# songrise/HyperNeRF-torch

Hardware: AMD Instinct MI355X
Metric: ray-samples/sec (fwd+bwd+Adam), whole job; per-GPU = value/n_gpus (higher is better)
Workload: dtype bf16

## Files before the change

### hypernerf-torch_amd/csrc/hn_mlp.hip

```cpp
#include "hn_common.h"
#include <algorithm>
#include <type_traits>

#ifdef HN_PROF
#define HN_STAMP(code)                                                                          \
  do {                                                                                          \
    if (prof_on && prof_n < 2040) {                                                             \
      unsigned long long t__;                                                                   \
      __builtin_amdgcn_sched_barrier(0);                                                        \
      asm volatile("s_memtime %0\n\ts_waitcnt lgkmcnt(0)" : "=s"(t__)::"memory");               \
      __builtin_amdgcn_sched_barrier(0);                                                        \
      if (lane == 0) { prof_buf[2 * prof_n] = (code); prof_buf[2 * prof_n + 1] = (long long)t__; } \
      ++prof_n;                                                                                 \
    }                                                                                           \
  } while (0)
#else
#define HN_STAMP(code) do {} while (0)
#endif

template <int WAVES>
struct WStream {
  const char* g;
  char* lds;
  int ctr;
// ... 463 lines not shown
#pragma unroll
  for (int t = 0; t <= NT; ++t) {
    const char* wl = nullptr;
    if (t < NT) wl = ws.take(N) + lane * 16;
    const int tp = t - 1;
    bf16x8 q[D];
    if (t < NT) {
      hn_init_acc(acc[t & 1], bias, t, h);
#pragma unroll
      for (int u = 0; u < D; ++u) q[u] = *reinterpret_cast<const bf16x8*>(wl + u * 1024);
    }
    __builtin_amdgcn_sched_barrier(0);
#pragma unroll
    for (int u = 0; u < N; ++u) {
      if (t < NT) {
        acc[t & 1] = hn_mfma_bf16(q[u % D], cur[u], acc[t & 1]);
        if (u + D < N) q[u % D] = *reinterpret_cast<const bf16x8*>(wl + (u + D) * 1024);
      }
      if (t > 0) {
#pragma unroll
        for (int e = 0; e < PER_SLOT; ++e) {
          const int k = u * PER_SLOT + e;
          if (k < SHARES)
            hn_epilogue_share<TRAIN, NT, S8>(k, tp, acc[tp & 1], nxt + tp * 2, bits, out_base, mask_base, lane);
        }
      }
      __builtin_amdgcn_sched_barrier(0);
    }
  }
#pragma unroll
  for (int i = 0; i < NT * 2; ++i) cur[i] = nxt[i];
}

template <bool BF16, int AUXG, bool EXTRA, bool TRAIN, bool S8 = false>
__global__ __launch_bounds__(ModeT<BF16>::WAVES * 64, BF16 ? 2 : 1) void hn_mlp_fwd_kernel(const HnMlpArgs a) {
  using M = ModeT<BF16>;
  constexpr int SX = S8 ? 1 : 0;
  static_assert(!(S8 && (EXTRA || !TRAIN || !BF16)), "the 8-bit stash exists for the render-level bf16 training builds only");
  if constexpr (S8) asm volatile("s_setreg_imm32_b32 hwreg(HW_REG_MODE, 23, 1), 1");
  using Frag = typename M::Frag;
  extern __shared__ __attribute__((aligned(16))) char smem[];
  const int lane = threadIdx.x & 63;
  const int wave = __builtin_amdgcn_readfirstlane(threadIdx.x >> 6);
  const int r = lane & 31, h = lane >> 5;
  constexpr int PTS = M::WAVES * 32;
  const int ntiles = (a.n_points + PTS - 1) / PTS;
  hn_timeline_begin(a.timeline);
#ifdef HN_PROF
  long long* prof_buf = reinterpret_cast<long long*>(a.prof);
  const bool prof_on = prof_buf != nullptr && blockIdx.x == 0 && wave == 0;
  int prof_n = 0;
#endif

  WStream<M::WAVES> ws;
  ws.g = reinterpret_cast<const char*>(a.wstream);
  ws.lds = smem;
  ws.nchunks = a.n_chunks;
  ws.wave = wave;
  ws.lane = lane;

  Frag cur[8 * M::STEPS32];
  Frag nxt[8 * M::STEPS32];

  float* bias_lds = reinterpret_cast<float*>(smem + 2 * HN_CHUNK_UNITS * 1024);
  HnFeat* feat_lds = reinterpret_cast<HnFeat*>(bias_lds + ((a.n_bias + 3) & ~3));
  HnDFeat* dfeat_lds = reinterpret_cast<HnDFeat*>(feat_lds + ((a.n_feat + 1) & ~1));
  const int n_trig = BF16 ? a.n_trig_comps : 0;
  const bool with_lo = a.trig_lo_planes != 0;
  const int n_planes = BF16 ? a.n_comps + n_trig + (with_lo ? n_trig : 1) : a.n_comps;
  float* srcv = reinterpret_cast<float*>(BF16 ? reinterpret_cast<char*>(dfeat_lds + a.n_feat)
                                              : reinterpret_cast<char*>(dfeat_lds)) + wave * (n_planes * 32);
  float* rev = BF16 ? srcv + a.n_comps * 32 : nullptr;
  for (int i = threadIdx.x; i < a.n_bias; i += blockDim.x) bias_lds[i] = a.bias[i];
  for (int i = threadIdx.x; i < a.n_feat; i += blockDim.x) {
    const HnFeat e = a.feat[i];
    feat_lds[i] = e;
    if constexpr (BF16) dfeat_lds[i] = hn_derive_feat_fwd(e, a.n_comps, n_trig, with_lo);
  }
  __syncthreads();

  for (int tile = blockIdx.x; tile < ntiles; tile += gridDim.x) {
    const int blk = tile * M::WAVES + wave;
    const int p0 = blk * 32 + r;
    const bool valid = p0 < a.n_points;
    const int p = valid ? p0 : a.n_points - 1;
    const int ray = p / a.samples_per_ray;
    const bool wave_valid = blk * 32 < a.n_points;
    hn_stage_sources(srcv, a, p, ray, lane, rev, n_trig, with_lo);
    ws.start();

    HnOpWords w_next = hn_load_op(a.ops, 0, a.n_ops);
    for (int op = 0; op < a.n_ops; ++op) {
      const HnOpWords w = w_next;
      w_next = hn_load_op(a.ops, op + 1, a.n_ops);
      const int code = w[0];
      if (code == HN_OP_LAYER) {
        HN_STAMP(100 + op);
        const int K32 = w[1] & 255, nG = (w[1] >> 8) & 255, NT = (w[1] >> 16) & 255;
        const int act = (w[1] >> 24) & 15, flags = (w[1] >> 28) & 15;
        const float* bias = bias_lds + w[2];
        const bool do_mask = TRAIN && w[4] >= 0 && wave_valid && act != HN_ACT_SOFTPLUS;
        const bool do_stash = TRAIN && w[5] >= 0 && wave_valid;
        char* out_base = do_stash ? hn_slot_base<BF16, SX>(a, w[5], NT, blk) : nullptr;
        char* aux_base = (TRAIN && wave_valid) ? hn_slot_base<BF16, SX>(a, w[6], 2 * nG, blk) : nullptr;
        uint32_t* mask_base = do_mask ? hn_mask_base(a, w[4], (NT + 1) >> 1, blk, lane) : nullptr;
        const bool has_out = w_next[0] == HN_OP_OUT;
        const HnOpWords out_w = w_next;
        Frag aux[AUXG * 2 * M::STEPS32];
#pragma unroll
        for (int g = 0; g < AUXG; ++g) {
          if (g < nG) {
            if (EXTRA && (flags & HN_LAYER_DIRECT))
              hn_make_group<true>(aux + g * 2 * M::STEPS32, feat_lds + w[3] + 64 * g, dfeat_lds + w[3] + 64 * g, srcv,
                                  lane, a, p, ray);
            else
              hn_make_group<false>(aux + g * 2 * M::STEPS32, feat_lds + w[3] + 64 * g, dfeat_lds + w[3] + 64 * g, srcv,
                                   lane, a, p, ray);
            if (aux_base != nullptr) {
              hn_stash<BF16, SX>(aux + g * 2 * M::STEPS32, aux_base, 2 * g, lane);
              hn_stash<BF16, SX>(aux + (g * 2 + 1) * M::STEPS32, aux_base, 2 * g + 1, lane);
            }
          }
        }
        unsigned bits = 0;
        HN_STAMP(1);
        if constexpr (BF16) {
          const bool plain = nG == 0 && act == HN_ACT_RELU && !(flags & HN_LAYER_NO_COMMIT) && !has_out &&
                             wave_valid && do_stash == do_mask;
          if (plain && K32 == 4 && NT == 4) {
            if (do_stash) hn_layer_pipelined<4, 4, true, SX>(cur, nxt, bias, ws, out_base, mask_base, lane);
            else hn_layer_pipelined<4, 4, false, SX>(cur, nxt, bias, ws, out_base, mask_base, lane);
            continue;
          }
        }
#pragma unroll
        for (int t = 0; t < 8; ++t) {
          if (t < NT) {
            f32x16 acc;
            hn_init_acc(acc, bias, t, h);
            hn_gemm_k<BF16>(acc, cur, K32, ws);
#pragma unroll
            for (int g = 0; g < AUXG; ++g)
              if (g < nG) hn_gemm_blocks<BF16, 2>(acc, aux + g * 2 * M::STEPS32, ws);
            HN_STAMP(2);
            if (act == HN_ACT_RELU) {
#pragma unroll
              for (int i = 0; i < 16; ++i) {
                bits = hn_push_mask<BF16>(bits, acc[i]);
                acc[i] = __int_as_float(max(__float_as_int(acc[i]), 0));
              }
            } else if (act != HN_ACT_NONE) {
              hn_act_tile<BF16>(acc, act, __int_as_float(w[7]), __int_as_float(w[4]), bits);
            }
            if (has_out && t == 0 && h == 0 && valid) {
              const HnDst d = a.dst[out_w[1]];
              const int n = out_w[3];
#pragma unroll
              for (int i = 0; i < 4; ++i) {
                if (i < n) {
                  float y = acc[i];
                  if (out_w[4] == 1) y = 1.0f / (1.0f + expf(-y));
                  if (out_w[5] >= 0) {
                    const HnSrc sr = a.src[out_w[5]];
                    y = __fadd_rn(sr.ptr[(size_t)(sr.per_ray ? ray : p) * sr.ld + out_w[6] + i], y);
                  }
                  d.ptr[(size_t)p * d.ld + out_w[2] + i] = y;
                }
              }
            }
            if (has_out && t == 0 && h == 0 && out_w[7] > 0) {
// ... 7 lines not shown
                    const HnSrc sr = a.src[out_w[5]];
                    y = __fadd_rn(sr.ptr[(size_t)(sr.per_ray ? ray : p) * sr.ld + out_w[6] + i], y);
                  }
                  const int ci = out_w[7] - 1 + i;
                  srcv[ci * 32 + r] = y;
                  if (BF16 && ci < n_trig) {
                    float hi, lo;
                    hn_rev_split(y, hi, lo);
                    rev[ci * 32 + r] = hi;
                    if (with_lo) rev[(n_trig + ci) * 32 + r] = lo;
                  }
                }
              }
            }
            hn_acc_to_frags(acc, nxt + t * M::STEPS32);
#ifdef HN_PROF
            if (prof_on) {
              float x__ = acc[15];
              asm volatile("v_mov_b32 %0, %0" : "+v"(x__)::"memory");
            }
#endif
            HN_STAMP(3);
            if ((t & 1) || t == NT - 1) {
              if (do_mask) mask_base[(t >> 1) * 64 + lane] = (t & 1) ? bits : bits << 16;
              bits = 0;
            }
            if (do_stash) {
              if constexpr (SX != 0) hn_stash8_acc<SX>(acc, out_base, t, lane);
              else hn_stash<BF16, SX>(nxt + t * M::STEPS32, out_base, t, lane);
            }
            HN_STAMP(4);
          }
        }
        if (!(flags & HN_LAYER_NO_COMMIT)) {
#pragma unroll
          for (int t = 0; t < 8; ++t)
            if (t < NT)
#pragma unroll
              for (int s = 0; s < M::STEPS32; ++s) cur[t * M::STEPS32 + s] = nxt[t * M::STEPS32 + s];
        }
      } else if (code == HN_OP_OUT) {
      } else if (EXTRA && code == HN_OP_OUT_WIDE) {
        const int n = w[3], NT = w[4];
        if (valid) {
          const HnDst d = a.dst[w[1]];
#pragma unroll
          for (int t = 0; t < 8; ++t)
            if (t < NT) {
              if constexpr (BF16) {
#pragma unroll
                for (int s = 0; s < 2; ++s)
#pragma unroll
                  for (int j = 0; j < 8; ++j) {
                    const int row = 32 * t + 16 * s + hn_pi16(h, j);
                    if (row < n) d.ptr[(size_t)p * d.ld + w[2] + row] = (float)cur[2 * t + s][j];
                  }
              } else {
#pragma unroll
                for (int q = 0; q < 16; ++q) {
                  const int row = 32 * t + hn_rho(q, h);
                  if (row < n) d.ptr[(size_t)p * d.ld + w[2] + row] = cur[16 * t + q];
                }
              }
            }
        }
      }
    }
  }
  hn_timeline_end(a.timeline);
}

HN_DEV bool hn_prefetch_masks(const HnMlpArgs& a, const HnOpWords& wn, int blk, int lane, bool wave_valid,
                              unsigned* out) {
  if (wn[0] != HN_BOP_LAYER || wn[4] < 0) return false;
  const int NT = (wn[1] >> 16) & 255;
  const uint32_t* mb = hn_mask_base(a, wn[4], (NT + 1) >> 1, blk, lane);
#pragma unroll
  for (int dd = 0; dd < 4; ++dd)
    out[dd] = (2 * dd < NT) ? (wave_valid ? mb[dd * 64 + lane] : 0xffffffffu) : 0u;
  return true;
}

template <bool BF16, bool WIDE, bool S8 = false>
__global__ __launch_bounds__(ModeT<BF16>::WAVES * 64, BF16 ? 2 : 1) void hn_mlp_bwd_kernel(const HnMlpArgs a) {
  using M = ModeT<BF16>;
  constexpr int SZ = S8 ? 2 : 0;
  static_assert(!(S8 && WIDE) && !(S8 && !BF16), "the 8-bit stash exists for the render-level bf16 builds only");
  if constexpr (S8) asm volatile("s_setreg_imm32_b32 hwreg(HW_REG_MODE, 23, 1), 1");
  const float dz_scale = S8 ? ldexpf(1.0f, a.dz_scale_log2) : 1.0f;
  const float dz_unscale = S8 ? ldexpf(1.0f, -a.dz_scale_log2) : 1.0f;
  using Frag = typename M::Frag;
  extern __shared__ __attribute__((aligned(16))) char smem[];
  const int lane = threadIdx.x & 63;
  const int wave = __builtin_amdgcn_readfirstlane(threadIdx.x >> 6);
  const int r = lane & 31, h = lane >> 5;
  constexpr int PTS = M::WAVES * 32;
  const int ntiles = (a.n_points + PTS - 1) / PTS;
  HnFeat* feat_lds = reinterpret_cast<HnFeat*>(smem + 2 * HN_CHUNK_UNITS * 1024);
  HnDFeat* dfeat_lds = reinterpret_cast<HnDFeat*>(feat_lds + ((a.n_feat + 1) & ~1));
  float* srcv = reinterpret_cast<float*>(BF16 ? reinterpret_cast<char*>(dfeat_lds + a.n_feat)
                                              : reinterpret_cast<char*>(dfeat_lds)) + wave * (a.n_comps * 32);
  hn_timeline_begin(a.timeline);
#ifdef HN_PROF
  long long* prof_buf = reinterpret_cast<long long*>(a.prof);
  const bool prof_on = prof_buf != nullptr && blockIdx.x == 0 && wave == 0;
  int prof_n = 0;
#endif
  for (int i = threadIdx.x; i < a.n_feat; i += blockDim.x) {
    const HnFeat e = a.feat[i];
    feat_lds[i] = e;
    if constexpr (BF16) dfeat_lds[i] = hn_derive_feat(e);
  }
  __syncthreads();

  WStream<M::WAVES> ws;
// ... 107 lines not shown
                float d = 1.0f;
                if (dact == HN_ACT_LEAKY_RELU) d = hn_keep_mask(nbits, t & 1, i) != 0 ? 1.0f : p0;
                else d = hn_dact_y<BF16>(dact, y[i], p0, p1);
                v[i] = g * d;
              }
            }
            hn_acc_to_frags(v, cur + t * M::STEPS32);
            if (dz_base != nullptr) hn_stash<BF16>(cur + t * M::STEPS32, dz_base, t, lane);
          }
        }
      } else if (code == HN_BOP_LAYER) {
        const int K32 = w[1] & 255, K32b = (w[1] >> 8) & 255, NT = (w[1] >> 16) & 255;
        const bool has_mask = w[4] >= 0;
        const bool do_stash = a.training && w[5] >= 0 && wave_valid;
        char* dz_base = do_stash ? hn_slot_base<BF16, SZ>(a, w[5], NT, blk) : nullptr;
        const int dact = w[2];
        const char* y_base = (!S8 && (dact == HN_ACT_ELU || dact == HN_ACT_SOFTPLUS) && wave_valid)
                                 ? hn_slot_base<BF16>(a, w[6], NT, blk) : nullptr;
        unsigned nbits = 0xffffffffu;
        unsigned mbits[4] = {0xffffffffu, 0xffffffffu, 0xffffffffu, 0xffffffffu};
        if (has_mask) {
          if (mnext_ready) {
#pragma unroll
            for (int dd = 0; dd < 4; ++dd) mbits[dd] = ~mnext[dd];
          } else {
            const uint32_t* mb = hn_mask_base(a, w[4], (NT + 1) >> 1, blk, lane);
#pragma unroll
            for (int dd = 0; dd < 4; ++dd)
              if (2 * dd < NT)
                mbits[dd] = wave_valid ? ~mb[dd * 64 + lane] : 0u;
          }
        }
        mnext_ready = false;
#pragma unroll
        for (int t = 0; t < 8; ++t) {
          if (t < NT) {
            f32x16 acc;
            hn_init_acc(acc, nullptr, t, h);
            hn_gemm_k<BF16>(acc, cur, K32, ws);
            if (K32b) hn_gemm_blocks<BF16, 1>(acc, cur2, ws);
            if (t == 0) mnext_ready = hn_prefetch_masks(a, w_next, blk, lane, wave_valid, mnext);
            HN_STAMP(2);
            if (!(t & 1)) nbits = mbits[t >> 1];
            if (dact == 0) {
#pragma unroll
              for (int i = 0; i < 16; ++i)
                acc[i] = __int_as_float(__float_as_int(acc[i]) & hn_keep_mask(nbits, t & 1, i));
            } else if (dact == HN_ACT_LEAKY_RELU) {
              const float p0 = __int_as_float(w[3]);
#pragma unroll
              for (int i = 0; i < 16; ++i)
                if (hn_keep_mask(nbits, t & 1, i) == 0) acc[i] *= p0;
            } else if (y_base != nullptr) {
              const f32x16 y = hn_unstash<BF16>(y_base, t, lane);
              const float p0 = __int_as_float(w[3]), p1 = __int_as_float(w[7]);
#pragma unroll
              for (int i = 0; i < 16; ++i) acc[i] *= hn_dact_y<BF16>(dact, y[i], p0, p1);
            }
            hn_acc_to_frags(acc, nxt + t * M::STEPS32);
            if (do_stash) {
              if constexpr (SZ != 0) hn_stash8_acc<SZ>(acc, dz_base, t, lane);
              else hn_stash<BF16, SZ>(nxt + t * M::STEPS32, dz_base, t, lane);
            }
            HN_STAMP(4);
          }
        }
// ... 569 lines not shown
    asm volatile("s_getreg_b32 %0, hwreg(HW_REG_HW_ID)" : "=s"(hw));
    asm volatile("s_getreg_b32 %0, hwreg(HW_REG_XCC_ID)" : "=s"(xcc));
    long long* o = jt_buf + (size_t)blockIdx.x * 8;
    o[0] = (long long)hw | ((long long)(xcc & 15u) << 32);
    o[1] = (long long)jt0; o[2] = (long long)jt1; o[3] = (long long)jt2; o[4] = (long long)wall_clock64();
    o[5] = (long long)nstage * (long long)stage_bytes; o[6] = jb.n_nt * 16 + jb.n_kt; o[7] = 1;
  }
#endif
  hn_timeline_end(tab.timeline);
}

static int hn_grid_for(int n_points, int pts_per_wg) {
  int tiles = (n_points + pts_per_wg - 1) / pts_per_wg;
  const int cap = 256 * 4;
  return tiles < cap ? tiles : cap;
}

extern "C" int hn_version(void) { return HN_VERSION; }

extern "C" int hn_abi_sizes(int32_t* out, int n) {
  const int32_t v[8] = {(int32_t)sizeof(HnMlpArgs),      (int32_t)sizeof(HnPackUnit), (int32_t)sizeof(HnPackBias),
                        (int32_t)sizeof(HnDwJob),        (int32_t)sizeof(HnCompositeArgs), (int32_t)sizeof(HnFeat),
                        (int32_t)sizeof(HnSlot),         (int32_t)sizeof(HnSrc)};
  static_assert(sizeof(HnDwBatch) == 40, "HnDwBatch layout");
  static_assert(sizeof(HnSrc) == 32, "HnSrc layout");
  for (int i = 0; i < n && i < 8; ++i) out[i] = v[i];
  return 8;
}

#define HN_STR2(x) #x
#define HN_STR(x) HN_STR2(x)
extern "C" __attribute__((used)) const char hn_build_config_text[] =
    "HN_BUILD_CONFIG:" HN_STR(HN_WGRAD_STAGES) "," HN_STR(HN_WGRAD_MAXSLOT) ",0," HN_STR(HN_CHUNK_UNITS) ",1,1,"
    HN_STR(HN_BF16_WAVES) "," HN_STR(HN_WGRAD_AUX) ";";
extern "C" int hn_build_config(int32_t* out, int n) {
  const int32_t v[HN_BUILD_CONFIG_N] = {HN_WGRAD_STAGES, HN_WGRAD_MAXSLOT, 0, HN_CHUNK_UNITS,
                                        1,               1,                HN_BF16_WAVES, HN_WGRAD_AUX};
  for (int i = 0; i < n && i < HN_BUILD_CONFIG_N; ++i) out[i] = v[i];
  return HN_BUILD_CONFIG_N;
}

static void hn_allow_big_lds() {
  static bool done[64] = {};
  int dev = 0;
  if (hipGetDevice(&dev) != hipSuccess || dev < 0 || dev >= 64) dev = 0;
  if (done[dev]) return;
  done[dev] = true;
  const int big = 160 * 1024;
#define HN_BIG(k) (void)hipFuncSetAttribute((const void*)(k), hipFuncAttributeMaxDynamicSharedMemorySize, big)
  HN_BIG((hn_mlp_fwd_kernel<true, 2, false, true>)); HN_BIG((hn_mlp_fwd_kernel<true, 2, false, false>));
  HN_BIG((hn_mlp_fwd_kernel<true, 2, true, true>)); HN_BIG((hn_mlp_fwd_kernel<true, 2, true, false>));
  HN_BIG((hn_mlp_fwd_kernel<true, 3, false, true>)); HN_BIG((hn_mlp_fwd_kernel<true, 3, false, false>));
  HN_BIG((hn_mlp_fwd_kernel<true, 3, true, true>)); HN_BIG((hn_mlp_fwd_kernel<true, 3, true, false>));
  HN_BIG((hn_mlp_fwd_kernel<false, 3, true, true>)); HN_BIG((hn_mlp_fwd_kernel<false, 3, true, false>));
  HN_BIG((hn_mlp_fwd_kernel<true, 2, false, true, true>)); HN_BIG((hn_mlp_fwd_kernel<true, 3, false, true, true>));
  HN_BIG((hn_mlp_bwd_kernel<true, false, true>)); HN_BIG((hn_wgrad_kernel<true, true>));
#undef HN_BIG
  (void)hipFuncSetAttribute((const void*)hn_mlp_bwd_kernel<true, false>, hipFuncAttributeMaxDynamicSharedMemorySize, big);
  (void)hipFuncSetAttribute((const void*)hn_mlp_bwd_kernel<true, true>, hipFuncAttributeMaxDynamicSharedMemorySize, big);
  (void)hipFuncSetAttribute((const void*)hn_mlp_bwd_kernel<false, true>, hipFuncAttributeMaxDynamicSharedMemorySize, big);
  (void)hipFuncSetAttribute((const void*)hn_wgrad_kernel<true>, hipFuncAttributeMaxDynamicSharedMemorySize, big);
  (void)hipFuncSetAttribute((const void*)hn_wgrad_kernel<false>, hipFuncAttributeMaxDynamicSharedMemorySize, big);
}

extern "C" int hn_pack_units(int mode, const HnPackUnit* units, int n_units, const float* const* ptrs, void* wstream,
                             const HnPackBias* bias, int n_bias, float* bias_out, hnStream_t stream) {
  if (n_units < 0 || n_bias < 0) return -1;
  const int total = n_units + n_bias;
  if (total == 0) return 0;
  const int grid = (total + 3) / 4;
// ... 530 lines not shown
```

### hypernerf-torch_amd/machine.py

```python
from __future__ import annotations

import os
import weakref

import ctypes as C
import itertools
import math
from dataclasses import dataclass, field
from typing import Dict, List, Optional, Sequence, Tuple

import numpy as np
import torch

from . import _lib as L

CHUNK = L.HN_CHUNK_UNITS


def pow2ceil(n: int) -> int:
    p = 1
    while p < n:
        p *= 2
    return p


def bf16_like(mode: int) -> bool:
    return mode in (L.HN_MODE_BF16, L.HN_MODE_BF16_S8)


def mode_consts(mode: int):
    if mode == L.HN_MODE_BF16_S8:
        return 2, 1024
    return (2, 2048) if mode == L.HN_MODE_BF16 else (4, 4096)


DZ_SCALE_LOG2 = int(os.environ.get("HN_DZ_SCALE_LOG2", 16))


ACT_CODES = {"none": L.HN_ACT_NONE, "relu": L.HN_ACT_RELU, "leaky_relu": L.HN_ACT_LEAKY_RELU, "elu": L.HN_ACT_ELU,
             "softplus": L.HN_ACT_SOFTPLUS}
MASK_ACTS = ("relu", "leaky_relu")
Y_ACTS = ("elu", "softplus")


def f32_bits(x: float) -> int:
    return int(np.array([x], dtype=np.float32).view(np.int32)[0])


@dataclass
class Feature:
    src: int
    comp: int
    kind: int
    freq: float = 1.0
    need_grad: bool = False


def posenc_features(src: int, comps: Sequence[int], n_freqs: int, need_grad: bool = False) -> List[Feature]:
    out = [Feature(src, c, L.HN_FEAT_ID, 1.0, need_grad) for c in comps]
    for k in range(n_freqs):
        f = float(2.0 ** k)
        out += [Feature(src, c, L.HN_FEAT_SIN, f, need_grad) for c in comps]
        out += [Feature(src, c, L.HN_FEAT_COS, f, need_grad) for c in comps]
    return out


def posenc_jax_features(src: int, comps: Sequence[int], min_deg: int, max_deg: int, use_identity: bool,
                        need_grad: bool = False) -> List[Feature]:
    steps = max_deg - min_deg
# ... 520 lines not shown
            if s.kind == "stash":
                offs.append((stash_b, s.nt))
                stash_b += nblk * s.nt * tile_bytes
            else:
                offs.append((mask_b, s.nt))
                mask_b += nblk * s.nt * 64 * 4
        return offs, stash_b, mask_b

    def resolved_ops(self, mode: int, n_points: int) -> Tuple[np.ndarray, np.ndarray]:
        offs, _, _ = self.layout(mode, n_points)

        def res(slot: int) -> int:
            if slot < 0:
                return -1
            off = offs[slot][0]
            unit = 1024 if self.slots[slot].kind == "stash" else 256
            assert off % unit == 0 and off // unit < 2 ** 31
            return off // unit
        fwd = self.fwd_ops.copy()
        for w in fwd:
            if w[0] == L.HN_OP_LAYER:
                if (int(w[1]) >> 24) & 15 != L.HN_ACT_SOFTPLUS:
                    w[4] = res(int(w[4]))
                w[5], w[6] = res(int(w[5])), res(int(w[6]))
        bwd = self.bwd_ops.copy()
        for w in bwd:
            if w[0] == L.HN_BOP_LOAD:
                w[7] = res(int(w[7]))
            elif w[0] == L.HN_BOP_LOAD_WIDE:
                if (int(w[3]) >> 16) & 15 != L.HN_ACT_SOFTPLUS:
                    w[5] = res(int(w[5]))
                w[7] = res(int(w[7]))
            elif w[0] == L.HN_BOP_LAYER:
                w[4], w[5] = res(int(w[4])), res(int(w[5]))
                if int(w[2]) in (L.HN_ACT_ELU, L.HN_ACT_SOFTPLUS):
                    w[6] = res(int(w[6]))
        return fwd, bwd

    def grad_offsets(self) -> Tuple[List[int], int]:
        offs, tot = [], 0
        for p in self.params:
            offs.append(tot)
            tot += (p.numel() + 3) // 4 * 4
        return offs, tot

    @staticmethod
    def _wave_grid(n_nt: int, n_kt: int, one_row: bool = False) -> Tuple[int, int]:
        if one_row:
            if n_nt <= 4:
                return 1, min(8, max(1, n_kt)) if n_kt <= 8 else 8
            return 2, 4
        best = None
        for gn in range(1, 9):
            for gk in range(1, 8 // gn + 1):
                if gn > n_nt or gk > n_kt:
                    continue
                tn, tk = -(-n_nt // gn), -(-n_kt // gk)
                if tn > 4 or tk > 2:
                    continue
                key = (-(gn * gk), tn * tk, gn * gk * (tn + tk))
                if best is None or key < best[0]:
                    best = (key, gn, gk)
        if best is None:
            raise NotImplementedError(f"no wave grid for a {n_nt} x {n_kt} tile rectangle")
        return best[1], best[2]

    def _wgrad_rects(self, mode: int, n_points: int) -> list:
        offs, _, _ = self.layout(mode, n_points)
        tmax = 8 if bf16_like(mode) else 4
        rects = []
        for ly in self.layers:
# ... 541 lines not shown
        a.masks = masks.data_ptr() if masks is not None else 0
        a.dsrc = dsrc.data_ptr() if dsrc is not None else 0
        for i, s in enumerate(srcs):
            if s is None:
                continue
            t, per_ray = s[0], s[1]
            L.require_gpu(t)
            if t.dtype != torch.float32 or t.stride(-1) != 1:
                raise L.HnError("sources must be fp32 with unit inner stride")
            a.src[i].ptr, a.src[i].ld, a.src[i].per_ray = t.data_ptr(), t.stride(-2) if t.dim() > 1 else 1, int(per_ray)
            if len(s) > 2 and s[2] is not None:
                idx = s[2]
                L.require_gpu(idx)
                if idx.dtype != torch.int64 or not idx.is_contiguous():
                    raise L.HnError("gather indices must be contiguous int64")
                a.src[i].gather_idx, a.src[i].gather_rows = idx.data_ptr(), t.shape[0]
        if embed is not None:
            g_tab, idx, src_i = embed[:3]
            if len(embed) > 3 and embed[3] is not None:
                a.embed_partial = embed[3].data_ptr()
            mask, col = self.prog.embed_fold(src_i)
            a.embed_reg_mask, a.embed_grad, a.embed_idx = mask, g_tab.data_ptr(), idx.data_ptr()
            a.embed_rows, a.embed_dim = g_tab.shape[0], g_tab.shape[1]
            for k in range(L.HN_DSRC_COMPS):
                a.embed_col[k] = col[k]
        for i, t in enumerate(dsts):
            if t is None:
                continue
            L.require_gpu(t)
            a.dst[i].ptr, a.dst[i].ld = t.data_ptr(), t.stride(-2) if t.dim() > 1 else 1
        return a

    def _ops(self, device, mode, n_points):
        key = ("ops", str(device), mode, n_points)
        hit = self._jobs.get(key)
        if hit is None:
            fwd, bwd = self.prog.resolved_ops(mode, n_points)
            hit = (L.to_device_bytes(fwd, device), L.to_device_bytes(bwd, device))
            self._jobs[key] = hit
        return hit

    @staticmethod
    def _job_bytes(mode: int) -> int:
        return WGRAD_JOB_BYTES // 2 if mode == L.HN_MODE_BF16_S8 else WGRAD_JOB_BYTES

    def effective_mode(self, mode: int) -> int:
        if mode == L.HN_MODE_BF16_S8:
            wide = any(ly.out is not None and ly.out.wide for ly in self.prog.layers)
            direct = any(f.kind != L.HN_FEAT_ZERO and (f.src, f.comp) not in self.prog.comp_map
                         for f in self.prog.feat_table)
            if wide or direct:
                return L.HN_MODE_BF16
        return mode

    def forward(self, mode, n_points, samples_per_ray, srcs, dsts, training: bool):
        mode = self.effective_mode(mode)
        if mode == L.HN_MODE_BF16_S8 and training and self.prog.y_acts:
            raise NotImplementedError(
                f"{self.prog.name}: precision 'bf16s8' keeps the training stash in 8 bits, too coarse to take the "
                "derivative of an ELU / Softplus layer from its output; use 'bf16' or 'fp32' (LeakyReLU works: it needs "
                "only the mask)")
        device = dsts[0].device if dsts and dsts[0] is not None else srcs[0][0].device
        d = self.pack(device, mode, force=training)
        stash = masks = None
        if training:
            _, sb, mb = self.prog.layout(mode, n_points)
            stash = torch.empty(max(sb, 16), dtype=torch.uint8, device=device)
# ... 67 lines not shown
```

### include/hn_kernels.h

```cpp
#ifndef HN_KERNELS_H
#define HN_KERNELS_H

#include <stdint.h>

#ifdef __cplusplus
extern "C" {
#endif

typedef void* hnStream_t;

#define HN_VERSION 340

#define HN_MODE_F32 0
#define HN_MODE_BF16 1
#define HN_MODE_BF16_S8 2

#define HN_MAX_SRC 8
#define HN_MAX_DST 4
#define HN_MAX_SLOTS 128
#define HN_OP_WORDS 8
#ifndef HN_CHUNK_UNITS
#define HN_CHUNK_UNITS 32
#endif
#define HN_DSRC_COMPS 32

#define HN_OP_LAYER 1
#define HN_ACT_NONE 0
#define HN_ACT_RELU 1
#define HN_ACT_LEAKY_RELU 2
#define HN_ACT_ELU 3
#define HN_ACT_SOFTPLUS 4
#define HN_LAYER_NO_COMMIT 1
#define HN_LAYER_DIRECT 2
#define HN_OP_OUT 4
#define HN_OP_OUT_WIDE 5

#define HN_BOP_LOAD 1
#define HN_BOP_LOAD_WIDE 2
#define HN_BOP_LAYER 3
#define HN_BOP_AUX 4

typedef struct {
  int32_t packed;
  float freq;
} HnFeat;
#define HN_MAX_COMPS 32
#define HN_FEAT_ID_DIRECT 5
#define HN_FEAT_ZERO 0
#define HN_FEAT_ID 1
#define HN_FEAT_SIN 2
#define HN_FEAT_COS 3
#define HN_FEAT_SINP 4

typedef struct {
  const float* ptr;
  int32_t ld;
  int32_t per_ray;
  const int64_t* gather_idx;
  int32_t gather_rows;
  int32_t pad;
} HnSrc;

typedef struct {
  float* ptr;
  int32_t ld;
  int32_t pad;
} HnDst;

typedef struct {
  uint64_t off;
  int32_t nt;
  int32_t pad;
// ... 43 lines not shown
  int32_t r_end;
  int32_t c_end;
  int32_t k0;
  int32_t transposed;
} HnPackUnit;

typedef struct {
  int32_t w_id;
  int32_t n;
  int32_t off;
  int32_t len;
} HnPackBias;

typedef struct {
  uint64_t z_off, x_off;
  int32_t z_nt, x_nt;
  int32_t z_t0, x_t0;
  int32_t n_nt, n_kt;
  int32_t blk0, blk1;
  int32_t w_off;
  int32_t ld;
  int32_t r0, c0;
  int32_t r_end, c_end;
  int32_t b_off;
  int32_t pad;
  uint64_t x2_off;
  int32_t x2_nt, x2_t0;
  int32_t n_kt1;
  int32_t p_tile;
} HnDwJob;

int hn_version(void);
int hn_abi_sizes(int32_t* out, int n);
#define HN_BUILD_CONFIG_N 8
int hn_build_config(int32_t* out, int n);

int hn_pack_units(int mode, const HnPackUnit* units_dev, int n_units, const float* const* ptrs_dev,
                  void* wstream_dev, const HnPackBias* bias_dev, int n_bias, float* bias_out_dev,
                  hnStream_t stream);

#define HN_MAX_PACK_JOBS 8
typedef struct {
  const HnPackUnit* units;
  const float* const* ptrs;
  void* wstream;
  const HnPackBias* bias;
  float* bias_out;
  int32_t n_units, n_bias;
} HnPackJob;
int hn_pack_units_multi(int mode, const HnPackJob* jobs_host, int n_jobs, hnStream_t stream);

int hn_mlp_forward(const HnMlpArgs* args, hnStream_t stream);
int hn_mlp_backward(const HnMlpArgs* args, hnStream_t stream);
int hn_mlp_workspace_bytes(const int32_t* ops_host, int n_ops, int backward, int mode, int64_t n_points,
                           int64_t* stash_bytes, int64_t* mask_bytes);

int hn_mlp_wgrad(int mode, const HnDwJob* jobs_dev, int n_jobs, const void* stash_dev,
                 float* grad_base_dev, hnStream_t stream);

#define HN_MAX_WGRAD_BATCH 8
typedef struct {
  const HnDwJob* jobs;
  const void* stash;
  float* grads;
  int32_t n_jobs;
  int32_t pad;
  float* partials;
// ... 206 lines not shown
```

### hypernerf-torch_amd/_lib.py

```python
from __future__ import annotations

import ctypes as C
import os
import subprocess

import numpy as np
import torch

_HERE = os.path.dirname(os.path.abspath(__file__))
CSRC = os.path.join(_HERE, "csrc")
PRODUCT_LIB_PATH = os.path.join(CSRC, "libhn_hip.so")
LIB_PATH = os.environ.get("HN_LIB_PATH") or PRODUCT_LIB_PATH
SOURCES = ["hn_mlp.hip", "hn_render.hip", "hn_calib.hip", "hn_optim.hip", "hn_metrics.hip"]
CSRC_HEADERS = ["hn_common.h", "hn_pack.h"]
HEADER = os.path.join(os.path.dirname(_HERE), "include", "hn_kernels.h")
BUILD_MACROS = ("HN_REDUCE_SPLIT", "HN_BF16_WAVES", "HN_PROF", "HN_CHUNK_UNITS", "HN_WGRAD_AUX", "HN_WGRAD_STAGES", "HN_WGRAD_MAXSLOT")

HN_MODE_F32, HN_MODE_BF16, HN_MODE_BF16_S8 = 0, 1, 2
BUILD_CONFIG_KEYS = ("WGRAD_STAGES", "WGRAD_MAXSLOT", "WGRAD_BIAS_MFMA", "CHUNK_UNITS", "WGRAD_BLOCK", "WSTREAM_ASYM",
                     "BF16_WAVES", "WGRAD_AUX")


def _read_build_config(path: str):
    import re
    try:
        with open(path, "rb") as f:
            blob = f.read()
    except OSError:
        return None
    m = re.search(rb"HN_BUILD_CONFIG:([0-9, ]+);", blob)
    if m is None:
        return None
    vals = [int(x) for x in m.group(1).decode().replace(" ", "").split(",")]
    return {k: v for k, v in zip(BUILD_CONFIG_KEYS, vals)}


BUILD_CONFIG = _read_build_config(LIB_PATH)
_cfg = BUILD_CONFIG or {}
WGRAD_STAGES = _cfg.get("WGRAD_STAGES", int(os.environ.get("HN_WGRAD_STAGES") or 2))
WGRAD_MAXSLOT = _cfg.get("WGRAD_MAXSLOT", int(os.environ.get("HN_WGRAD_MAXSLOT") or 8))
WGRAD_MAX_STAGE_KB = min(8 * WGRAD_MAXSLOT, 160 // WGRAD_STAGES)
HN_MAX_SRC, HN_MAX_DST, HN_MAX_SLOTS = 8, 4, 128
HN_OP_WORDS, HN_CHUNK_UNITS, HN_DSRC_COMPS = 8, _cfg.get("CHUNK_UNITS", int(os.environ.get("HN_CHUNK_UNITS", 32))), 32
HN_AUXG_MAX = 3
HN_MAX_COMPS = 32

HN_OP_LAYER, HN_OP_OUT, HN_OP_OUT_WIDE = 1, 4, 5
HN_ACT_NONE, HN_ACT_RELU, HN_ACT_LEAKY_RELU, HN_ACT_ELU, HN_ACT_SOFTPLUS = 0, 1, 2, 3, 4
HN_LAYER_NO_COMMIT, HN_LAYER_DIRECT = 1, 2
HN_BOP_LOAD, HN_BOP_LOAD_WIDE, HN_BOP_LAYER, HN_BOP_AUX = 1, 2, 3, 4
HN_FEAT_ZERO, HN_FEAT_ID, HN_FEAT_SIN, HN_FEAT_COS, HN_FEAT_SINP, HN_FEAT_ID_DIRECT = 0, 1, 2, 3, 4, 5


# ... 281 lines not shown
```

Measured before the change: 83.62 million.

## Software-pipeline backward ReLU layer epilogue with next tile's MFMA chain

Adds a specialized backward path for bf16 layers with K32=4, NT=4, ReLU-style masking (dact=0) and stashing. Each tile's mask, bf16 conversion and stash epilogue is interleaved with the next tile's MFMA chain, using double-buffered accumulators and a two-deep weight prefetch, with sched_barriers to fix the ordering. The intent is to hide epilogue ALU and LDS/global latency behind matrix-core work. The trade-off is higher register pressure, and an env var plus an op flag bit let the path be disabled.

```diff
diff --git a/hypernerf-torch_amd/csrc/hn_mlp.hip b/hypernerf-torch_amd/csrc/hn_mlp.hip
--- a/hypernerf-torch_amd/csrc/hn_mlp.hip
+++ b/hypernerf-torch_amd/csrc/hn_mlp.hip
@@ -745,6 +745,65 @@
   return true;
 }
 
+template <bool TRAIN, int SZ>
+HN_DEV void hn_bwd_epilogue_share(int k, int tp, f32x16& a, bf16x8* frag, unsigned nbits, char* dz_base, int lane) {
+  if (k < 8) {
+#pragma unroll
+    for (int e = 0; e < 2; ++e) {
+      const int i = 2 * k + e;
+      a[i] = __int_as_float(__float_as_int(a[i]) & hn_keep_mask(nbits, tp & 1, i));
+      frag[i >> 3][i & 7] = (__bf16)a[i];
+    }
+  } else if (TRAIN && k == 8) {
+    if constexpr (SZ != 0) hn_stash8_acc<SZ>(a, dz_base, tp, lane);
+    else hn_stash<true, 0>(frag, dz_base, tp, lane);
+  }
+}
+
+template <int K32, int NT, bool TRAIN, int SZ>
+HN_DEV bool hn_bwd_layer_pipelined(bf16x8* cur, bf16x8* nxt, const unsigned* mbits, WStream<ModeT<true>::WAVES>& ws,
+                                   char* dz_base, const HnMlpArgs& a, const HnOpWords& w_next, int blk, int lane,
+                                   unsigned* mnext) {
+  constexpr int N = 2 * K32;
+  constexpr int D = 2;
+  static_assert(8 % N == 0, "the eight element-pair shares are dealt evenly over the slots");
+  constexpr int PER_SLOT = 8 / N;
+  f32x16 acc[2];
+  bool mnext_ready = false;
+#pragma unroll
+  for (int t = 0; t <= NT; ++t) {
+    const char* wl = nullptr;
+    if (t < NT) wl = ws.take(N) + lane * 16;
+    if (t == 0) mnext_ready = hn_prefetch_masks(a, w_next, blk, lane, true, mnext);
+    const int tp = t - 1;
+    bf16x8 q[D];
+    if (t < NT) {
+      hn_init_acc(acc[t & 1], nullptr, t, 0);
+#pragma unroll
+      for (int u = 0; u < D; ++u) q[u] = *reinterpret_cast<const bf16x8*>(wl + u * 1024);
+    }
+    __builtin_amdgcn_sched_barrier(0);
+#pragma unroll
+    for (int u = 0; u < N; ++u) {
+      if (t < NT) {
+        acc[t & 1] = hn_mfma_bf16(q[u % D], cur[u], acc[t & 1]);
+        if (u + D < N) q[u % D] = *reinterpret_cast<const bf16x8*>(wl + (u + D) * 1024);
+      }
+      if (t > 0) {
+#pragma unroll
+        for (int e = 0; e < PER_SLOT; ++e)
+          hn_bwd_epilogue_share<TRAIN, SZ>(u * PER_SLOT + e, tp, acc[tp & 1], nxt + tp * 2, mbits[tp >> 1], dz_base, lane);
+        if (u == N - 1)
+          hn_bwd_epilogue_share<TRAIN, SZ>(8, tp, acc[tp & 1], nxt + tp * 2, mbits[tp >> 1], dz_base, lane);
+      }
+      __builtin_amdgcn_sched_barrier(0);
+    }
+  }
+#pragma unroll
+  for (int i = 0; i < NT * 2; ++i) cur[i] = nxt[i];
+  return mnext_ready;
+}
+
 template <bool BF16, bool WIDE, bool S8 = false>
 __global__ __launch_bounds__(ModeT<BF16>::WAVES * 64, BF16 ? 2 : 1) void hn_mlp_bwd_kernel(const HnMlpArgs a) {
   using M = ModeT<BF16>;
@@ -918,6 +977,12 @@
           }
         }
         mnext_ready = false;
+        if constexpr (BF16) {
+          if (!(w[1] & HN_BOP_GENERIC_ONLY) && K32b == 0 && dact == 0 && wave_valid && do_stash && K32 == 4 && NT == 4) {
+            mnext_ready = hn_bwd_layer_pipelined<4, 4, true, SZ>(cur, nxt, mbits, ws, dz_base, a, w_next, blk, lane, mnext);
+            continue;
+          }
+        }
 #pragma unroll
         for (int t = 0; t < 8; ++t) {
           if (t < NT) {
diff --git a/hypernerf-torch_amd/machine.py b/hypernerf-torch_amd/machine.py
--- a/hypernerf-torch_amd/machine.py
+++ b/hypernerf-torch_amd/machine.py
@@ -35,6 +35,9 @@
 
 
 DZ_SCALE_LOG2 = int(os.environ.get("HN_DZ_SCALE_LOG2", 16))
+
+BWD_PIPELINE = os.environ.get("HN_BWD_PIPE", "1") != "0"
+BOP_GENERIC_ONLY = -(1 << 31)
 
 
 ACT_CODES = {"none": L.HN_ACT_NONE, "relu": L.HN_ACT_RELU, "leaky_relu": L.HN_ACT_LEAKY_RELU, "elu": L.HN_ACT_ELU,
@@ -621,6 +624,8 @@
                     w[5] = res(int(w[5]))
                 w[7] = res(int(w[7]))
             elif w[0] == L.HN_BOP_LAYER:
+                if not BWD_PIPELINE:
+                    w[1] = int(w[1]) | BOP_GENERIC_ONLY
                 w[4], w[5] = res(int(w[4])), res(int(w[5]))
                 if int(w[2]) in (L.HN_ACT_ELU, L.HN_ACT_SOFTPLUS):
                     w[6] = res(int(w[6]))
@@ -1233,7 +1238,7 @@
         return a
 
     def _ops(self, device, mode, n_points):
-        key = ("ops", str(device), mode, n_points)
+        key = ("ops", str(device), mode, n_points, BWD_PIPELINE)
         hit = self._jobs.get(key)
         if hit is None:
             fwd, bwd = self.prog.resolved_ops(mode, n_points)
diff --git a/include/hn_kernels.h b/include/hn_kernels.h
--- a/include/hn_kernels.h
+++ b/include/hn_kernels.h
@@ -38,6 +38,7 @@
 #define HN_BOP_LOAD 1
 #define HN_BOP_LOAD_WIDE 2
 #define HN_BOP_LAYER 3
+#define HN_BOP_GENERIC_ONLY ((int)0x80000000)
 #define HN_BOP_AUX 4
 
 typedef struct {
```

Result: no change. 83.43 million (-0.2%).

## Add specialized fused trunk-layer paths for 256x256 ReLU layers in fwd and bwd

Applied to the files above, without the earlier changes.

Adds dedicated device routines for the common 8x8-tile ReLU trunk layers in the MLP forward and backward kernels. In the forward pass, two consecutive trunk layers run back to back with ping-pong buffers, so the copy between them is skipped. In the backward pass, a specialized masked-gradient loop replaces the generic one. The path is gated by a build macro that defaults on, and the macro is recorded in the build config. Costs include more code size and register pressure, which could hurt occupancy.

```diff
diff --git a/hypernerf-torch_amd/_lib.py b/hypernerf-torch_amd/_lib.py
--- a/hypernerf-torch_amd/_lib.py
+++ b/hypernerf-torch_amd/_lib.py
@@ -14,11 +14,11 @@
 SOURCES = ["hn_mlp.hip", "hn_render.hip", "hn_calib.hip", "hn_optim.hip", "hn_metrics.hip"]
 CSRC_HEADERS = ["hn_common.h", "hn_pack.h"]
 HEADER = os.path.join(os.path.dirname(_HERE), "include", "hn_kernels.h")
-BUILD_MACROS = ("HN_REDUCE_SPLIT", "HN_BF16_WAVES", "HN_PROF", "HN_CHUNK_UNITS", "HN_WGRAD_AUX", "HN_WGRAD_STAGES", "HN_WGRAD_MAXSLOT")
+BUILD_MACROS = ("HN_REDUCE_SPLIT", "HN_BF16_WAVES", "HN_PROF", "HN_CHUNK_UNITS", "HN_WGRAD_AUX", "HN_WGRAD_STAGES", "HN_WGRAD_MAXSLOT", "HN_TRUNK_BODY")
 
 HN_MODE_F32, HN_MODE_BF16, HN_MODE_BF16_S8 = 0, 1, 2
 BUILD_CONFIG_KEYS = ("WGRAD_STAGES", "WGRAD_MAXSLOT", "WGRAD_BIAS_MFMA", "CHUNK_UNITS", "WGRAD_BLOCK", "WSTREAM_ASYM",
-                     "BF16_WAVES", "WGRAD_AUX")
+                     "BF16_WAVES", "WGRAD_AUX", "TRUNK_BODY")
 
 
 def _read_build_config(path: str):
diff --git a/hypernerf-torch_amd/csrc/hn_mlp.hip b/hypernerf-torch_amd/csrc/hn_mlp.hip
--- a/hypernerf-torch_amd/csrc/hn_mlp.hip
+++ b/hypernerf-torch_amd/csrc/hn_mlp.hip
@@ -519,6 +519,65 @@
   for (int i = 0; i < NT * 2; ++i) cur[i] = nxt[i];
 }
 
+#ifndef HN_TRUNK_BODY
+#define HN_TRUNK_BODY 1
+#endif
+typedef __attribute__((ext_vector_type(8))) short hn_s16x8;
+template <bool TRAIN>
+HN_DEV bool hn_trunk_fwd_op(const HnOpWords& w, const HnOpWords& wn) {
+  constexpr int shape = 8 | 0 << 8 | 8 << 16 | HN_ACT_RELU << 24;
+  return w[0] == HN_OP_LAYER && (w[1] & 0x1fffffff) == shape && wn[0] != HN_OP_OUT &&
+         (!TRAIN || (w[4] >= 0) == (w[5] >= 0));
+}
+HN_DEV bool hn_trunk_bwd_op(const HnOpWords& w) {
+  return w[0] == HN_BOP_LAYER && w[1] == (8 | 8 << 16) && w[2] == 0 && w[4] >= 0;
+}
+template <bool TRAIN, int S8>
+HN_DEV void hn_trunk_fwd(const bf16x8* in, bf16x8* out, const float* bias, WStream<ModeT<true>::WAVES>& ws, bool store,
+                         char* out_base, uint32_t* mask_base, int lane) {
+  asm volatile("" : "+v"(lane));
+  const int h = lane >> 5;
+  unsigned bits = 0;
+#pragma unroll
+  for (int t = 0; t < 8; ++t) {
+    f32x16 acc;
+    hn_init_acc(acc, bias, t, h);
+    hn_gemm_blocks<true, 8>(acc, in, ws);
+    if constexpr (TRAIN) {
+#pragma unroll
+      for (int i = 0; i < 16; ++i) bits = hn_push_mask<true>(bits, acc[i]);
+    }
+#pragma unroll
+    for (int i = 0; i < 16; ++i) acc[i] = __int_as_float(max(__float_as_int(acc[i]), 0));
+    hn_acc_to_frags(acc, out + 2 * t);
+    if (TRAIN && store) {
+      if constexpr (S8 != 0) hn_stash8_acc<S8>(acc, out_base, t, lane);
+      else hn_stash<true, 0>(out + 2 * t, out_base, t, lane);
+    }
+    if (TRAIN && store && (t & 1)) mask_base[(t >> 1) * 64 + lane] = bits;
+  }
+}
+template <int S8, class F>
+HN_DEV void hn_trunk_bwd(const bf16x8* in, bf16x8* out, WStream<ModeT<true>::WAVES>& ws, const unsigned* mbits,
+                         bool store, char* dz_base, int lane, F&& after_first) {
+  asm volatile("" : "+v"(lane));
+#pragma unroll
+  for (int t = 0; t < 8; ++t) {
+    f32x16 acc;
+    hn_init_acc(acc, nullptr, t, 0);
+    hn_gemm_blocks<true, 8>(acc, in, ws);
+    if (t == 0) after_first();
+    const unsigned nbits = mbits[t >> 1];
+#pragma unroll
+    for (int i = 0; i < 16; ++i) acc[i] = __int_as_float(__float_as_int(acc[i]) & hn_keep_mask(nbits, t & 1, i));
+    hn_acc_to_frags(acc, out + 2 * t);
+    if (store) {
+      if constexpr (S8 != 0) hn_stash8_acc<S8>(acc, dz_base, t, lane);
+      else hn_stash<true, 0>(out + 2 * t, dz_base, t, lane);
+    }
+  }
+}
+
 template <bool BF16, int AUXG, bool EXTRA, bool TRAIN, bool S8 = false>
 __global__ __launch_bounds__(ModeT<BF16>::WAVES * 64, BF16 ? 2 : 1) void hn_mlp_fwd_kernel(const HnMlpArgs a) {
   using M = ModeT<BF16>;
@@ -566,12 +625,19 @@
   }
   __syncthreads();
 
+  constexpr bool TRUNK = HN_TRUNK_BODY && BF16 && TRAIN && !EXTRA && !S8 && AUXG == 2;
   for (int tile = blockIdx.x; tile < ntiles; tile += gridDim.x) {
+    int spr = a.samples_per_ray;
+    if constexpr (TRUNK) {
+      asm volatile("" : "+s"(spr));
+      asm volatile("v_mbcnt_lo_u32_b32 %0, -1, 0\n\tv_mbcnt_hi_u32_b32 %0, -1, %0" : "=&v"(ws.lane));
+    }
+    const int lane = ws.lane, r = lane & 31, h = lane >> 5;
     const int blk = tile * M::WAVES + wave;
     const int p0 = blk * 32 + r;
     const bool valid = p0 < a.n_points;
     const int p = valid ? p0 : a.n_points - 1;
-    const int ray = p / a.samples_per_ray;
+    const int ray = p / spr;
     const bool wave_valid = blk * 32 < a.n_points;
     hn_stage_sources(srcv, a, p, ray, lane, rev, n_trig, with_lo);
     ws.start();
@@ -620,9 +686,27 @@
             continue;
           }
         }
+        bool trunk = false, swapped = false;
+        if constexpr (TRUNK) {
+          trunk = wave_valid && hn_trunk_fwd_op<TRAIN>(w, w_next);
+          if (trunk) {
+            const HnOpWords w2 = hn_load_op(a.ops, op + 2, a.n_ops);
+            hn_trunk_fwd<TRAIN, SX>(cur, nxt, bias, ws, do_stash, out_base, mask_base, lane);
+            if (hn_trunk_fwd_op<TRAIN>(w_next, w2)) {
+              const bool st2 = TRAIN && w_next[5] >= 0;
+              char* ob2 = st2 ? hn_slot_base<true, SX>(a, w_next[5], 8, blk) : nullptr;
+              uint32_t* mb2 = st2 ? hn_mask_base(a, w_next[4], 4, blk, lane) : nullptr;
+              HN_STAMP(100 + op + 1);
+              hn_trunk_fwd<TRAIN, SX>(nxt, cur, bias_lds + w_next[2], ws, st2, ob2, mb2, lane);
+              ++op;
+              w_next = w2;
+              swapped = true;
+            }
+          }
+        }
 #pragma unroll
         for (int t = 0; t < 8; ++t) {
-          if (t < NT) {
+          if (t < NT && !trunk) {
             f32x16 acc;
             hn_init_acc(acc, bias, t, h);
             hn_gemm_k<BF16>(acc, cur, K32, ws);
@@ -696,7 +780,7 @@
             HN_STAMP(4);
           }
         }
-        if (!(flags & HN_LAYER_NO_COMMIT)) {
+        if (!(flags & HN_LAYER_NO_COMMIT) && !swapped) {
 #pragma unroll
           for (int t = 0; t < 8; ++t)
             if (t < NT)
@@ -918,6 +1002,17 @@
           }
         }
         mnext_ready = false;
+#if HN_TRUNK_BODY
+        if constexpr (BF16) {
+          if (hn_trunk_bwd_op(w)) {
+            hn_trunk_bwd<SZ>(cur, nxt, ws, mbits, do_stash, dz_base, lane,
+                             [&] { mnext_ready = hn_prefetch_masks(a, w_next, blk, lane, wave_valid, mnext); });
+#pragma unroll
+            for (int i = 0; i < 16; ++i) cur[i] = nxt[i];
+            continue;
+          }
+        }
+#endif
 #pragma unroll
         for (int t = 0; t < 8; ++t) {
           if (t < NT) {
@@ -1553,10 +1648,11 @@
 #define HN_STR(x) HN_STR2(x)
 extern "C" __attribute__((used)) const char hn_build_config_text[] =
     "HN_BUILD_CONFIG:" HN_STR(HN_WGRAD_STAGES) "," HN_STR(HN_WGRAD_MAXSLOT) ",0," HN_STR(HN_CHUNK_UNITS) ",1,1,"
-    HN_STR(HN_BF16_WAVES) "," HN_STR(HN_WGRAD_AUX) ";";
+    HN_STR(HN_BF16_WAVES) "," HN_STR(HN_WGRAD_AUX) "," HN_STR(HN_TRUNK_BODY) ";";
 extern "C" int hn_build_config(int32_t* out, int n) {
   const int32_t v[HN_BUILD_CONFIG_N] = {HN_WGRAD_STAGES, HN_WGRAD_MAXSLOT, 0, HN_CHUNK_UNITS,
-                                        1,               1,                HN_BF16_WAVES, HN_WGRAD_AUX};
+                                        1,               1,                HN_BF16_WAVES, HN_WGRAD_AUX,
+                                        HN_TRUNK_BODY};
   for (int i = 0; i < n && i < HN_BUILD_CONFIG_N; ++i) out[i] = v[i];
   return HN_BUILD_CONFIG_N;
 }
diff --git a/hypernerf-torch_amd/machine.py b/hypernerf-torch_amd/machine.py
--- a/hypernerf-torch_amd/machine.py
+++ b/hypernerf-torch_amd/machine.py
@@ -626,6 +626,30 @@
                     w[6] = res(int(w[6]))
         return fwd, bwd
 
+    def trunk_body_ops(self) -> Tuple[List[Tuple[int, str]], List[Tuple[int, str]]]:
+        def walk(ops, is_trunk):
+            out, op, n = [], 0, len(ops)
+            word = lambda i: ops[i] if i < n else [-1] * L.HN_OP_WORDS
+            while op < n:
+                if is_trunk(word(op), word(op + 1)):
+                    if is_trunk(word(op + 1), word(op + 2)):
+                        out += [(op, "first"), (op + 1, "second")]
+                        op += 2
+                        continue
+                    out.append((op, "copy"))
+                op += 1
+            return out
+
+        shape = 8 | 8 << 16 | L.HN_ACT_RELU << 24
+
+        def fwd_trunk(w, wn):
+            return int(w[0]) == L.HN_OP_LAYER and (int(w[1]) & 0x1fffffff) == shape and int(wn[0]) != L.HN_OP_OUT \
+                and (int(w[4]) >= 0) == (int(w[5]) >= 0)
+
+        def bwd_trunk(w, wn):
+            return int(w[0]) == L.HN_BOP_LAYER and int(w[1]) == (8 | 8 << 16) and int(w[2]) == 0 and int(w[4]) >= 0
+        return walk(self.fwd_ops.tolist(), fwd_trunk), walk(self.bwd_ops.tolist(), bwd_trunk)
+
     def grad_offsets(self) -> Tuple[List[int], int]:
         offs, tot = [], 0
         for p in self.params:
diff --git a/include/hn_kernels.h b/include/hn_kernels.h
--- a/include/hn_kernels.h
+++ b/include/hn_kernels.h
@@ -147,7 +147,7 @@
 
 int hn_version(void);
 int hn_abi_sizes(int32_t* out, int n);
-#define HN_BUILD_CONFIG_N 8
+#define HN_BUILD_CONFIG_N 9
 int hn_build_config(int32_t* out, int n);
 
 int hn_pack_units(int mode, const HnPackUnit* units_dev, int n_units, const float* const* ptrs_dev,
```

After: 80.53 million before, 79.77 million after. About the same (-0.9%).
